# githubpradeep/llm_np_cp

Measured on AMD Instinct MI355X. Metric: decode tokens/sec, higher is better.
Workload: dtype bf16; 1 GPU; model=llama-3.2-1b, kv_dtype=bf16, global_batch=1, seq_len=867, parallelism=tp1

## Files before the change

### csrc/llm_ops.hip

```cpp

#include <hip/hip_runtime.h>
#include <cstdint>
#include <cstdio>
#include <cstdlib>
#include <type_traits>

#include "common.h"


#define GEMV_ROWS_PER_BLOCK 4
#define STAGE_RAW 0
#define STAGE_NORM 1
#define STAGE_GLU 2
#define STAGE_NORM2 3
#define STAGE_NORM_EMBED 4

DEVINL u16 glu_act(float xx, float u, int act) {
  float a;
  if (act == 0) {
    a = xx / (1.f + __expf(-xx));
  } else {
    float c = 0.7978845608028654f * (xx + 0.044715f * xx * xx * xx);
    a = 0.5f * xx * (1.f + tanhf(c));
  }
// ... 1605 lines not shown
        if (mnew != -INFINITY) mrun = mnew;
        kv = kvn; vv = vvn; kraw = krawn; vraw = vrawn;
        valid = validn; ksc = kscn; vsc = vscn;
      }
    }
  }

  for (int w = LP; w < 64; w <<= 1) {
    float mo = __shfl_xor(mrun, w);
    float lo = __shfl_xor(lrun, w);
    float mn = fmaxf(mrun, mo);
    float sa = (mrun == -INFINITY && mo == -INFINITY) ? 0.f : __expf(mrun - mn);
    float sb = (mrun == -INFINITY && mo == -INFINITY) ? 0.f : __expf(mo - mn);
#pragma unroll
    for (int j = 0; j < 8; j++) {
      float ao = __shfl_xor(acc[j], w);
      acc[j] = acc[j] * sa + ao * sb;
    }
    lrun = lrun * sa + lo * sb;
    mrun = mn;
  }

  float* accs = red;
  float* mls = red + 4 * hd;
  if (lane < LP) {
#pragma unroll
    for (int j = 0; j < 8; j++) accs[wave * hd + d0 + j] = acc[j];
  }
  if (lane == 0) {
    mls[wave * 2] = mrun;
    mls[wave * 2 + 1] = lrun;
  }
  __syncthreads();
  if (wave == 0) {
    float mt = fmaxf(fmaxf(mls[0], mls[2]), fmaxf(mls[4], mls[6]));
    float lt = 0.f, sc[4];
#pragma unroll
    for (int w = 0; w < 4; w++) {
      sc[w] = (mls[w * 2] == -INFINITY) ? 0.f : __expf(mls[w * 2] - mt);
      lt += mls[w * 2 + 1] * sc[w];
    }
    float inv = 1.f / lt;
    for (int d = lane; d < hd; d += 64) {
      float v = 0.f;
#pragma unroll
      for (int w = 0; w < 4; w++) v += accs[w * hd + d] * sc[w];
      out[((size_t)m * nh + h) * hd + d] = f2b(v * inv);
    }
  }
}


template <bool KV8>
__global__ void __launch_bounds__(256)
k_attn_dec_t(const u16* __restrict__ qkv, void* __restrict__ kc,
             void* __restrict__ vc, u16* __restrict__ out,
             const int* __restrict__ len_ptr, const float* __restrict__ cost,
             const float* __restrict__ sint, float* __restrict__ kS,
             float* __restrict__ vS, float* __restrict__ scratch,
             int* __restrict__ cnt, int nh, int kvh, int hd, int S,
             float scale, float softcap, int window) {
  extern __shared__ __attribute__((aligned(16))) char smem[];
  float* red = (float*)smem;
  int* lastflag = (int*)(red + 4 * hd + 8);

  const int h = blockIdx.x;
  const int chunk = blockIdx.y, SPLIT = gridDim.y;
  const int b = blockIdx.z;
  qkv += (size_t)b * (nh + 2 * kvh) * hd;
  out += (size_t)b * nh * hd;
  kc = (char*)kc + (size_t)b * kvh * S * hd * (KV8 ? 1 : 2);
  vc = (char*)vc + (size_t)b * kvh * S * hd * (KV8 ? 1 : 2);
  if (KV8) { kS += (size_t)b * kvh * S; vS += (size_t)b * kvh * S; }
  scratch += (size_t)b * nh * SPLIT * (hd + 2);
  cnt += b * nh;
  const int grp = nh / kvh;
  const int kvhead = h / grp;
  const int pos = len_ptr[b];
  int start = 0;
  if (window > 0 && pos + 1 - window > 0) start = pos + 1 - window;
  const int hist = pos - start;
  const int clen = (hist + SPLIT - 1) / SPLIT;
  const int c0 = start + chunk * clen;
  const int c1 = min(c0 + clen, pos);
  const bool last_chunk = (chunk == SPLIT - 1);

  const int LP = hd / 8;
  const int PP = 64 / LP;
  const int wave = threadIdx.x >> 6, lane = threadIdx.x & 63;
  const int p = lane / LP, d0 = (lane % LP) * 8;
  const int hd2 = hd / 2;
  const float* cp = cost + (size_t)pos * hd2;
  const float* sp = sint + (size_t)pos * hd2;

  const u16* qh = qkv + (size_t)h * hd;
  const u16* kh = qkv + (size_t)(nh + kvhead) * hd;
  const u16* vh = qkv + (size_t)(nh + kvh + kvhead) * hd;
  const u16* K0 = (const u16*)kc + (size_t)kvhead * S * hd;
  const u16* V0 = (const u16*)vc + (size_t)kvhead * S * hd;
  const uint8_t* K08 = (const uint8_t*)kc + (size_t)kvhead * S * hd;
  const uint8_t* V08 = (const uint8_t*)vc + (size_t)kvhead * S * hd;
  const float* kS0 = KV8 ? kS + (size_t)kvhead * S : nullptr;
  const float* vS0 = KV8 ? vS + (size_t)kvhead * S : nullptr;

  auto ldkv = [&](int tt, bool& vld, s8v& ko, s8v& vo,
                  unsigned long long& kro, unsigned long long& vro,
                  float& kso, float& vso) {
    vld = false;
    if (tt < c1) {
      int t_ = tt + p;
      vld = t_ < c1;
      int tl_ = vld ? t_ : c0;
      if (KV8) {
        kro = *(const unsigned long long*)(K08 + (size_t)tl_ * hd + d0);
        vro = *(const unsigned long long*)(V08 + (size_t)tl_ * hd + d0);
        kso = kS0[tl_]; vso = vS0[tl_];
      } else {
        ko = *(const s8v*)(K0 + (size_t)tl_ * hd + d0);
        vo = *(const s8v*)(V0 + (size_t)tl_ * hd + d0);
      }
// ... 190 lines not shown
    } else {
      for (int d = lane; d < hd; d += 64) {
        float v = 0.f;
#pragma unroll
        for (int w = 0; w < 4; w++) v += accs[w * hd + d] * sc[w];
        part[2 + d] = v;
      }
      if (lane == 0) { part[0] = mt; part[1] = lt; }
    }
  }
  if (SPLIT == 1) return;

  asm volatile("s_waitcnt vmcnt(0)" ::: "memory");
  __syncthreads();
  if (threadIdx.x == 0) {
    __builtin_amdgcn_fence(__ATOMIC_RELEASE, "agent");
    asm volatile("s_waitcnt vmcnt(0)" ::: "memory");
    int t = __hip_atomic_fetch_add(&cnt[h], 1, __ATOMIC_RELAXED,
                                   __HIP_MEMORY_SCOPE_AGENT);
    *lastflag = (t == SPLIT - 1);
  }
  __syncthreads();
  if (!*lastflag) return;

  if (threadIdx.x == 0)
    __builtin_amdgcn_fence(__ATOMIC_ACQUIRE, "agent");
  __syncthreads();
  if (wave == 0) {
    const float* base = scratch + (size_t)h * SPLIT * (hd + 2);
    float mt = -INFINITY;
    for (int c = 0; c < SPLIT; c++)
      mt = fmaxf(mt, base[(size_t)c * (hd + 2)]);
    float lt = 0.f;
    for (int c = 0; c < SPLIT; c++) {
      float mc = base[(size_t)c * (hd + 2)];
      if (mc != -INFINITY)
        lt += base[(size_t)c * (hd + 2) + 1] * __expf(mc - mt);
    }
    float inv = 1.f / lt;
    for (int d = lane; d < hd; d += 64) {
      float v = 0.f;
      for (int c = 0; c < SPLIT; c++) {
        float mc = base[(size_t)c * (hd + 2)];
        if (mc != -INFINITY)
          v += base[(size_t)c * (hd + 2) + 2 + d] * __expf(mc - mt);
      }
      out[(size_t)h * hd + d] = f2b(v * inv);
    }
  }
  __syncthreads();
  if (threadIdx.x == 0) cnt[h] = 0;
}

extern "C" hipError_t launch_attn_dec(const void* qkv, void* kc, void* vc,
                                      void* out, const void* len_ptr,
                                      const void* cost, const void* sint,
                                      void* kS, void* vS, int kv8,
                                      void* scratch, void* cnt, int split,
                                      int batch,
                                      int nh, int kvh, int hd, int S,
                                      float scale, float softcap, int window,
                                      hipStream_t stream) {
  size_t lds = (4 * hd + 8) * sizeof(float) + 16;
#define ATTN_DEC_CASE(KV8V)                                                  \
  hipLaunchKernelGGL((k_attn_dec_t<KV8V>), dim3(nh, split, batch),          \
                     dim3(256), lds,                                        \
                     stream, (const u16*)qkv, kc, vc, (u16*)out,            \
                     (const int*)len_ptr, (const float*)cost,               \
                     (const float*)sint, (float*)kS, (float*)vS,            \
                     (float*)scratch, (int*)cnt, nh, kvh, hd, S, scale,     \
                     softcap, window)
  if (kv8) ATTN_DEC_CASE(true);
  else ATTN_DEC_CASE(false);
#undef ATTN_DEC_CASE
  return hipGetLastError();
}


typedef short b4v __attribute__((ext_vector_type(4)));

template <int HD, bool KV8>
__global__ void __launch_bounds__(64)
k_attn_prefill_mfma(const u16* __restrict__ q, const void* __restrict__ kc,
                    const void* __restrict__ vc, u16* __restrict__ out,
                    const int* __restrict__ len_ptr,
                    const float* __restrict__ kS,
                    const float* __restrict__ vS, int M, int nh, int kvh,
                    int S, float scale, float softcap, int window) {
  constexpr int HD32 = HD / 32;
  constexpr int HD16 = HD / 16;
  const int h = blockIdx.x;
  const int qt = blockIdx.y;
  const int kvhead = h / (nh / kvh);
  const int pos0 = *len_ptr;
  const int lane = threadIdx.x & 63;
  const int qcol = lane & 15;
  const int krow4 = (lane >> 4) * 4;

  const int m0 = qt * 16;
  const int my_m = m0 + qcol;
  const int qpos = pos0 + my_m;

  s8v qf[HD32];
  {
    int mr = my_m < M ? my_m : M - 1;
    const u16* qp = q + ((size_t)mr * nh + h) * HD;
#pragma unroll
    for (int c = 0; c < HD32; c++)
      qf[c] = *(const s8v*)(qp + c * 32 + (lane >> 4) * 8);
  }

  const u16* K0 = (const u16*)kc + (size_t)kvhead * S * HD;
  const u16* V0 = (const u16*)vc + (size_t)kvhead * S * HD;
  const uint8_t* K08 = (const uint8_t*)kc + (size_t)kvhead * S * HD;
  const uint8_t* V08 = (const uint8_t*)vc + (size_t)kvhead * S * HD;
  const float* kS0 = KV8 ? kS + (size_t)kvhead * S : nullptr;
  const float* vS0 = KV8 ? vS + (size_t)kvhead * S : nullptr;

  float mrun = -INFINITY, lrun = 0.f;
  f4v acc_o[HD16];
#pragma unroll
  for (int d = 0; d < HD16; d++) acc_o[d] = {0.f, 0.f, 0.f, 0.f};

  __shared__ u16 vlds[16 * HD];
  const int T_end = min(pos0 + M, pos0 + m0 + 16);
  int t_start = 0;
  if (window > 0) {
    t_start = pos0 + m0 + 1 - window;
// ... 1571 lines not shown
#pragma unroll
  for (int i = 0; i < 4; i++) {
#pragma unroll
    for (int j = 0; j < 4; j++) {
#pragma unroll
      for (int r = 0; r < 4; r++) {
        int row = bm + wrow * 64 + i * 16 + cr + r;
        int col = bn + wcol * 64 + j * 16 + cc;
        if (row < M && col < N) {
          float v = acc[i][j][r];
          if (SK > 1) {
            atomicAdd(accbuf + (size_t)row * N + col, v);
          } else {
            if (res) v += b2f(res[(size_t)row * N + col]);
            Y[(size_t)row * N + col] = f2b(v);
          }
        }
      }
    }
  }
}

extern "C" hipError_t launch_gemm_fp4w(const void* X, const void* W4,
                                       const void* WE, void* Y,
                                       const void* res, void* accbuf, int M,
                                       int N, int K, hipStream_t stream) {
  if (K % 64 != 0) return hipErrorInvalidValue;
  int gm = (M + BM - 1) / BM, gn = (N + BN - 1) / BN;
  int sk = 1;
  if (accbuf && gm * gn < 160) {
    while (sk < 8 && gm * gn * sk * 2 <= 512 && (K / BK) % (sk * 2) == 0)
      sk *= 2;
  }
  if (sk > 1) {
    long total = (long)M * N;
    hipLaunchKernelGGL(k_zero_f32, dim3((uint32_t)((total + 1023) / 1024)),
                       dim3(256), 0, stream, (float*)accbuf, total);
  }
  dim3 grid(gm, gn, sk);
  hipLaunchKernelGGL(k_gemm_fp4w, grid, dim3(256), 0, stream, (const u16*)X,
                     (const uint8_t*)W4, (const uint8_t*)WE, (u16*)Y,
                     (const u16*)res, (float*)accbuf, M, N, K);
  if (sk > 1) {
    long total = (long)M * N;
    hipLaunchKernelGGL(k_gemm_fin, dim3((uint32_t)((total + 255) / 256)),
                       dim3(256), 0, stream, (const float*)accbuf,
                       (const u16*)res, (u16*)Y, total);
  }
  return hipGetLastError();
}


extern "C" __global__ void __launch_bounds__(256)
k_prefetch(const u16* __restrict__ p, long n, float* __restrict__ sink) {
  float acc = 0.f;
  for (long i = ((long)blockIdx.x * 256 + threadIdx.x) * 8; i < n;
       i += (long)gridDim.x * 256 * 8) {
    s8v v = *(const s8v*)(p + i);
    acc += b2f(((u16*)&v)[0]);
  }
  if (acc == 1e30f) sink[blockIdx.x] = acc;
}

extern "C" hipError_t launch_prefetch(const void* p, long n_elems,
                                      void* sink, hipStream_t stream) {
  hipLaunchKernelGGL(k_prefetch, dim3(128), dim3(256), 0, stream,
                     (const u16*)p, n_elems, (float*)sink);
  return hipGetLastError();
}


extern "C" __global__ void __launch_bounds__(256)
k_softcap(u16* __restrict__ y, long total, float cap) {
  long i = ((long)blockIdx.x * 256 + threadIdx.x) * 8;
  if (i >= total) return;
  s8v v = *(const s8v*)(y + i);
  u16 o[8];
#pragma unroll
  for (int j = 0; j < 8; j++)
    o[j] = f2b(cap * tanhf(b2f(((u16*)&v)[j]) / cap));
  *(s8v*)(y + i) = *(s8v*)o;
}

extern "C" hipError_t launch_softcap(void* y, long total, float cap,
                                     hipStream_t stream) {
  long blocks = (total / 8 + 255) / 256;
  hipLaunchKernelGGL(k_softcap, dim3((uint32_t)blocks), dim3(256), 0, stream,
                     (u16*)y, total, cap);
  return hipGetLastError();
}


extern "C" __global__ void __launch_bounds__(256)
k_bias_add(u16* __restrict__ y, const u16* __restrict__ bias, long total,
           int N) {
  long i = ((long)blockIdx.x * 256 + threadIdx.x) * 8;
  if (i >= total) return;
  s8v yv = *(const s8v*)(y + i);
  s8v bv = *(const s8v*)(bias + (i % N));
  u16 o[8];
#pragma unroll
  for (int j = 0; j < 8; j++)
    o[j] = f2b(b2f(((u16*)&yv)[j]) + b2f(((u16*)&bv)[j]));
  *(s8v*)(y + i) = *(s8v*)o;
}

extern "C" hipError_t launch_bias_add(void* y, const void* bias, int M,
                                      int N, hipStream_t stream) {
  if (N % 8 != 0) return hipErrorInvalidValue;
  long total = (long)M * N;
  hipLaunchKernelGGL(k_bias_add, dim3((uint32_t)((total / 8 + 255) / 256)),
                     dim3(256), 0, stream, (u16*)y, (const u16*)bias, total,
                     N);
  return hipGetLastError();
}


extern "C" __global__ void __launch_bounds__(256)
k_addinto(u16* __restrict__ y, const u16* __restrict__ a, long total) {
  long i = ((long)blockIdx.x * 256 + threadIdx.x) * 8;
  if (i >= total) return;
  s8v yv = *(const s8v*)(y + i);
  s8v av = *(const s8v*)(a + i);
  u16 o[8];
#pragma unroll
// ... 179 lines not shown
```

### llm_np_cp_amd/models/engine.py

```python

from __future__ import annotations

from typing import Dict, Optional

import numpy as np
import torch

from ..core.config import ModelConfig
from ..ops import hip_ops as ho
from ..parallel import tp as tpu
from ..utils.tracing import trace_range


class DeviceCacheHandle:

    def __init__(self, engine):
        self.engine = engine
        self.seq_len = 0


class GPUModel:
    device_strategies = frozenset(
        {"greedy", "min_p", "top_k", "top_p", "temperature"})
    device_processors = frozenset()
# ... 36 lines not shown
                {"logit_bias", "repetition_penalty", "frequency_penalty",
                 "presence_penalty"})
        self.p_stat = self.p_proc = self.p_bias = None
        self._proc_rows = {}
        if self.world == 1:
            self.device_logprobs = ho.LOGPROBS_MAX_TOP
        self.lp_cfg = self.lp_stage = self.lp_part = None
        self.lp_val = self.lp_idx = self.lp_raw = None
        self._lp_rows = {}
        self._lp_batch = False
        self.last_logprobs = None
        if self.world == 1:
            self.device_row_sampler = True
        self._samp_modes = {}
        self._req_serial = 0
        self._s_rows = frozenset({0})
        if device is None:
            device = f"cuda:{self.rank % max(torch.cuda.device_count(), 1)}"
        self.device = torch.device(device)
        torch.cuda.set_device(self.device)

        cfg = config
        tp = self.world
        assert cfg.num_attention_heads % tp == 0, "nh must divide tp"
        assert cfg.num_key_value_heads % tp == 0, \
            f"kv heads {cfg.num_key_value_heads} not divisible by tp {tp}"
        assert cfg.intermediate_size % tp == 0
        assert cfg.vocab_size % tp == 0
        if self.moe and tp > 1:
            raise ValueError("MoE tensor parallelism (expert parallel) "
                             "is not implemented yet — run TP=1")
        self.nh_l = cfg.num_attention_heads // tp
        self.kvh_l = cfg.num_key_value_heads // tp
        self.inter_l = cfg.intermediate_size // tp
        self.vocab_l = cfg.vocab_size // tp
        self.hd = cfg.head_dim
        self.H = cfg.hidden_size

        if self.world > 1:
            slot_bytes = max(self.H * 2, self.vocab_l * 4, 1 << 16)
            tpu.init_xgmi(self.device, slot_bytes)
        import torch.distributed as dist
        self._async_ar = bool(
            self.world > 1 and dist.is_initialized()
            and "nccl" in str(dist.get_backend()).lower())

        self._upload_weights(weights)
        if max_seq is None:
            max_seq = self._auto_max_seq()
        self.max_seq = max_seq
        self._alloc_state(prefill_chunk)
        self._graph = None
        self._graph_mode = None
        import os as _os
        self.prefetch_on = _os.environ.get("LLM_PREFETCH", "0") == "1"
        self._pf_stream = torch.cuda.Stream(device=self.device)
        self._pf_sink = torch.zeros(256, dtype=torch.float32,
                                    device=self.device)
        self._pf_events = []

    def _auto_max_seq(self) -> int:
        cfg = self.config
        free, _total = torch.cuda.mem_get_info(self.device)
        esz = 1 if self.kv8 else 2
        per_pos = (cfg.num_hidden_layers * self.kvh_l * self.hd * 2 * esz
                   * self.max_batch)
        if self.kv8:
            per_pos += (cfg.num_hidden_layers * self.kvh_l * 2 * 4
                        * self.max_batch)
        per_pos += self.hd * 4 + 8
        budget = int(free * 0.9) - (2 << 30)
        n = max(1024, budget // max(per_pos, 1))
        return int(min(cfg.max_position_embeddings, n))

    def _upload_weights(self, w: Dict[str, np.ndarray]):
        from ..io.loader import validate_weights

        validate_weights(self.config, w)
        cfg, dev = self.config, self.device
        tp, r = self.world, self.rank
        gemma = cfg.model_type == "gemma2"

        def bf16(a: np.ndarray) -> torch.Tensor:
            return torch.from_numpy(np.ascontiguousarray(a)).to(
                dev, torch.bfloat16, non_blocking=False)

        def gamma(a: np.ndarray) -> torch.Tensor:
            g = a.astype(np.float32) + (1.0 if gemma else 0.0)
            return torch.from_numpy(g).to(dev)

        def quant4(a: np.ndarray):
            t = bf16(a)
            N, K = t.shape
            q = torch.empty(N, K // 2, dtype=torch.uint8, device=dev)
            e = torch.empty(N, K // 32, dtype=torch.uint8, device=dev)
            ho.quant_fp4(t, q, e)
            torch.cuda.synchronize()
            return q, e

        def quant8(a: np.ndarray):
            t = bf16(a)
            N, K = t.shape
            q = torch.empty(N, K, dtype=torch.uint8, device=dev)
            s = torch.empty(N, dtype=torch.float32, device=dev)
            ho.quant_fp8(t, q, s)
            torch.cuda.synchronize()
            return q, s

        self.embed = bf16(w["model.embed_tokens.weight"])
        lm_w = w.get("lm_head.weight", w["model.embed_tokens.weight"])
        if self.fp8:
            lmw = lm_w if tp == 1 else tpu.shard_rows(lm_w, r, tp)
# ... 800 lines not shown
                if on_ids:
                    on_ids(take)
                if stop:
                    break
                if stop_fn is not None and stop_fn(out):
                    break
        if logprobs is not None:
            N = int(logprobs)
            self.last_logprobs = (
                np.concatenate([r[0] for r in recs]) if recs
                else np.zeros(0, np.float32),
                np.concatenate([r[1] for r in recs]) if recs
                else np.zeros((0, N), np.int32),
                np.concatenate([r[2] for r in recs]) if recs
                else np.zeros((0, N), np.float32))
        return out

    def forward(self, ids: np.ndarray, cache: DeviceCacheHandle,
                pos0: int) -> np.ndarray:
        ids = np.asarray(ids, dtype=np.int32).ravel()
        if pos0 != cache.seq_len:
            raise ValueError("GPU engine requires sequential positions")
        n = len(ids)
        if n == 0:
            raise ValueError("empty ids")
        if pos0 + n > self.max_seq:
            raise ValueError(f"sequence {pos0}+{n} exceeds max_seq "
                             f"{self.max_seq}")
        done = 0
        while done < n:
            M = min(n - done, self.PC)
            self.ids_buf[:M].copy_(
                torch.from_numpy(ids[done:done + M].astype(np.int32)))
            ho.i32_set(self.len_buf, pos0 + done)
            ho.embed(self.embed, self.ids_buf, self.b_h, M,
                     self.config.embed_scale)
            self._layers_forward(M)
            done += M
        ho.i32_set(self.len_buf, pos0 + n)
        self._host_len = pos0 + n
        self._lm_head_last(M)
        cache.seq_len = pos0 + n
        torch.cuda.synchronize()
        return self.b_logits.float().cpu().numpy()[None, :]

    def _dgemv(self, lw, name, x, y, **kw):
        if self.wq4:
            ho.gemv_fp4(lw[name + "_q4"], lw[name + "_e4"], x, y, **kw)
        elif self.fp8:
            ho.gemv_fp8(lw[name + "_q"], lw[name + "_s"], x, y, **kw)
        else:
            ho.gemv(lw[name], x, y, **kw)

    def _pf_tensors(self, lw):
        if self.wq4:
            return (lw["wqkv_q4"], lw["wo_q4"], lw["wgu_q4"],
                    lw["wdown_q4"])
        if self.fp8:
            return (lw["wqkv_q"], lw["wo_q"], lw["wgu_q"], lw["wdown_q"])
        return (lw["wqkv"], lw["wo"], lw["wgu"], lw["wdown"])

    def _decode_step(self, greedy: bool, min_p: float,
                     temperature: float = 1.0, top_k: int = 0,
                     top_p: float = 1.0, proc: bool = False,
                     logprobs: bool = False, rows=None):
        cfg = self.config
        eps = cfg.rms_norm_eps
        if self.fp8 or self.wq4:
            gukw = {}
            downkw = dict(stage=ho.STAGE_GLU, x2=self.b_gu[self.inter_l:],
                          act=self.act)
        else:
            gukw = dict(glu_pair=True, act=self.act)
            downkw = {}
        h = self.b_h[0]
        hnext = self.b_hb
        t1 = self.b_t1[0]
        t2 = self.b_t2
        s0 = torch.cuda.current_stream()
        pf = self.prefetch_on
        self._pf_events = []
        prev = None
        for i, lw in enumerate(self.layers):
            if pf and i + 1 < len(self.layers):
                ev = torch.cuda.Event()
                ev.record(s0)
                self._pf_events.append(ev)
                self._pf_stream.wait_event(ev)
                with torch.cuda.stream(self._pf_stream):
                    for t in self._pf_tensors(self.layers[i + 1]):
                        ho.prefetch(t, self._pf_sink)
            window = cfg.sliding_window if cfg.is_sliding(i) else 0
            if self.gemma and prev is not None:
                self._dgemv(lw, "wqkv", t2, self.b_qkv,
                            stage=ho.STAGE_NORM2, x2=h,
                            g=prev["g_postffn"], g2=lw["g_in"], res=hnext,
                            eps=eps)
                h, hnext = hnext, h
            elif i == 0 and "bqkv" not in lw:
                self._dgemv(lw, "wqkv", self.embed, self.b_qkv,
                            stage=ho.STAGE_NORM_EMBED, x2=self.next_token,
                            g=lw["g_in"], res=h, eps=eps,
                            escale=cfg.embed_scale)
            else:
                if i == 0:
                    ho.embed(self.embed, self.next_token, self.b_h, 1,
                             cfg.embed_scale)
                self._dgemv(lw, "wqkv", h, self.b_qkv, stage=ho.STAGE_NORM,
                            g=lw["g_in"], res=lw.get("bqkv"), eps=eps)
            prev = lw
            ho.attn_dec(self.b_qkv, self.k_cache[i], self.v_cache[i],
                        self.b_att[0], self.len_buf, self.cos_t, self.sin_t,
                        self.attn_scratch, self.attn_cnt,
                        self.nh_l, self.kvh_l, self.hd, self.scale,
                        softcap=self.attn_softcap, window=window or 0,
                        split=self.attn_split,
                        kS=self.k_scale[i], vS=self.v_scale[i])
            if self.gemma:
                self._dgemv(lw, "wo", self.b_att[0], t1)
                tpu.all_reduce(t1)
                self._dgemv(lw, "wgu", t1, self.b_gu, stage=ho.STAGE_NORM2,
                            x2=h, g=lw["g_post"], g2=lw["g_preffn"],
                            res=hnext, eps=eps, **gukw)
                h, hnext = hnext, h
                self._dgemv(lw, "wdown", self.b_gu[:self.inter_l], t2,
                            **downkw)
                tpu.all_reduce(t2)
            else:
                if self.tp_branch:
                    self._dgemv(lw, "wo", self.b_att[0], t1)
                    tpu.all_reduce(t1)
                    ho.addinto(h, t1)
                else:
                    self._dgemv(lw, "wo", self.b_att[0], h, res=h)
                if self.moe:
                    ho.moe_route(h, lw["g_post"], lw["wg"], 1, self.topk,
                                 self.moe_idx, self.moe_w, eps=eps)
                    xn0 = self.b_xn[0]
                    ho.rmsnorm(h, lw["g_post"], xn0, eps=eps)
                    I, H = self.inter_l, self.H
                    for j in range(self.topk):
                        ei = self.moe_idx[j:j + 1]
                        osc = self.moe_w[j:j + 1]
                        if self.fp8:
                            ho.gemv_fp8(lw["wgu_q"], lw["wgu_s"], xn0,
                                        self.b_gu, eidx=ei,
                                        wstride=2 * I * H, sstride=2 * I)
                            ho.gemv_fp8(lw["wdown_q"], lw["wdown_s"],
                                        self.b_gu[:I], h, res=h,
                                        stage=ho.STAGE_GLU,
                                        x2=self.b_gu[I:], act=self.act,
                                        eidx=ei, wstride=H * I,
                                        sstride=H, oscale=osc)
                        else:
                            ho.gemv(lw["wgu"], xn0, self.b_gu, eidx=ei,
                                    wstride=2 * I * H)
                            ho.gemv(lw["wdown"], self.b_gu[:I], h, res=h,
                                    stage=ho.STAGE_GLU, x2=self.b_gu[I:],
                                    act=self.act, eidx=ei,
                                    wstride=H * I, oscale=osc)
                    continue
                self._dgemv(lw, "wgu", h, self.b_gu, stage=ho.STAGE_NORM,
                            g=lw["g_post"], eps=eps, **gukw)
                if self.tp_branch:
                    self._dgemv(lw, "wdown", self.b_gu[:self.inter_l], t1,
                                **downkw)
                    tpu.all_reduce(t1)
                    ho.addinto(h, t1)
                else:
                    self._dgemv(lw, "wdown", self.b_gu[:self.inter_l], h,
                                res=h, **downkw)
        if pf:
            ev = torch.cuda.Event()
            ev.record(self._pf_stream)
            self._pf_events.append(ev)
            s0.wait_event(ev)
        if self.gemma:
            kw = dict(stage=ho.STAGE_NORM2, x2=h,
                      g=self.layers[-1]["g_postffn"], g2=self.g_final,
                      res=hnext, eps=eps, softcap=self.final_softcap)
            if self.wq4:
                ho.gemv_fp4(self.lm_head_q4, self.lm_head_e4, t2,
                            self.b_logits_l, **kw)
            elif self.fp8:
                ho.gemv_fp8(self.lm_head_q, self.lm_head_s, t2,
                            self.b_logits_l, **kw)
            else:
                ho.gemv(self.lm_head, t2, self.b_logits_l, **kw)
        else:
            kw = dict(stage=ho.STAGE_NORM, g=self.g_final, eps=eps,
                      softcap=self.final_softcap)
            if self.wq4:
                ho.gemv_fp4(self.lm_head_q4, self.lm_head_e4, h,
                            self.b_logits_l, **kw)
            elif self.fp8:
                ho.gemv_fp8(self.lm_head_q, self.lm_head_s, h,
                            self.b_logits_l, **kw)
            else:
                ho.gemv(self.lm_head, h, self.b_logits_l, **kw)
        if self.tp_branch:
            tpu.all_gather_into(self.b_logits, self.b_logits_l)
        if logprobs:
            self._lp_scan(self.b_logits, slice(0, 1), proc)
        if proc:
            ho.logit_adjust(self.b_logits, self.p_stat, self.p_proc,
                            self.p_bias, self.next_token, True)
        self._sample_step(greedy, min_p, temperature, top_k, top_p, rows)
        if logprobs:
            self._lp_commit(self.b_logits, slice(0, 1), proc,
                            self.next_token, self.nout)

    def _decode_batch_step(self, B: int, greedy: bool, min_p: float,
                           temperature: float = 1.0, top_k: int = 0,
                           top_p: float = 1.0, proc: bool = False,
                           logprobs: bool = False, rows=None):
        cfg = self.config
        import os as _os
        mx_max = int(_os.environ.get("LLM_BATCH_MX_MAX", "0"))
        if (self.fp8 and B <= mx_max and not cfg.attention_bias
                and not self.moe):
            return self._decode_batch_step_mx(B, greedy, min_p, temperature,
                                              top_k, top_p, proc, logprobs,
                                              rows)
        if self.fp8 and B <= 16 and not self.moe:
            return self._decode_batch_step_skinny(B, greedy, min_p,
                                                  temperature, top_k,
                                                  top_p, proc, logprobs,
                                                  rows)
        ho.embed(self.embed, self.bt_next, self.b_h, B, cfg.embed_scale)
# ... 604 lines not shown
```

### llm_np_cp_amd/ops/hip_ops.py

```python

from __future__ import annotations

import ctypes
import os

import numpy as np
import torch

_LIB = None
_LIB_PATH = os.path.join(os.path.dirname(os.path.dirname(
    os.path.abspath(__file__))), "_libllmops.so")

_SIGS = {
    "launch_gemv_bf16": [ctypes.c_void_p] * 7 + [ctypes.c_int] * 4 +
                        [ctypes.c_float, ctypes.c_int, ctypes.c_float,
                         ctypes.c_int, ctypes.c_int, ctypes.c_int,
                         ctypes.c_float, ctypes.c_void_p, ctypes.c_long,
                         ctypes.c_void_p, ctypes.c_void_p, ctypes.c_int],
    "launch_gemv_fp8": [ctypes.c_void_p] * 8 + [ctypes.c_int] * 4 +
                       [ctypes.c_float, ctypes.c_int, ctypes.c_float,
                        ctypes.c_int, ctypes.c_int, ctypes.c_int,
                        ctypes.c_float, ctypes.c_void_p, ctypes.c_long,
                        ctypes.c_long, ctypes.c_void_p, ctypes.c_void_p],
    "launch_rmsnorm": [ctypes.c_void_p] * 4 + [ctypes.c_int] * 2 +
                      [ctypes.c_float, ctypes.c_int, ctypes.c_void_p],
    "launch_rope_cache": [ctypes.c_void_p] * 7 + [ctypes.c_int] +
                         [ctypes.c_void_p] * 3 + [ctypes.c_int] * 5 +
                         [ctypes.c_void_p],
    "launch_attn": [ctypes.c_void_p] * 7 + [ctypes.c_int] * 6 +
                   [ctypes.c_float, ctypes.c_float, ctypes.c_int,
                    ctypes.c_void_p],
    "launch_attn_prefill_mfma": [ctypes.c_void_p] * 7 + [ctypes.c_int] * 6 +
                                [ctypes.c_float, ctypes.c_float,
                                 ctypes.c_int, ctypes.c_void_p],
    "launch_attn_dec": [ctypes.c_void_p] * 9 + [ctypes.c_int] +
                       [ctypes.c_void_p] * 2 + [ctypes.c_int] * 6 +
                       [ctypes.c_float, ctypes.c_float, ctypes.c_int,
                        ctypes.c_void_p],
    "launch_glu": [ctypes.c_void_p] * 3 + [ctypes.c_long, ctypes.c_int,
                                           ctypes.c_void_p],
    "launch_embed": [ctypes.c_void_p] * 3 + [ctypes.c_int] * 2 +
                    [ctypes.c_float, ctypes.c_void_p],
    "launch_sample": [ctypes.c_void_p, ctypes.c_int, ctypes.c_int,
                      ctypes.c_int, ctypes.c_long, ctypes.c_float,
                      ctypes.c_int, ctypes.c_uint64, ctypes.c_float] +
                     [ctypes.c_void_p] * 8 +
                     [ctypes.c_int, ctypes.c_void_p],
    "launch_sample_sel": [ctypes.c_void_p, ctypes.c_int, ctypes.c_int,
                          ctypes.c_int, ctypes.c_long, ctypes.c_float,
                          ctypes.c_int, ctypes.c_uint64, ctypes.c_float] +
                         [ctypes.c_void_p] * 8 +
                         [ctypes.c_int, ctypes.c_int, ctypes.c_float,
                          ctypes.c_void_p, ctypes.c_void_p],
    "launch_sample_rows": [ctypes.c_void_p, ctypes.c_int, ctypes.c_int,
                           ctypes.c_int, ctypes.c_long, ctypes.c_void_p,
                           ctypes.c_int, ctypes.c_int] +
                          [ctypes.c_void_p] * 7 +
                          [ctypes.c_int, ctypes.c_void_p, ctypes.c_void_p],
    "launch_logit_adjust": [ctypes.c_void_p, ctypes.c_int, ctypes.c_int,
                            ctypes.c_int] + [ctypes.c_void_p] * 4 +
                           [ctypes.c_int, ctypes.c_void_p],
    "launch_tokstat_mark": [ctypes.c_void_p, ctypes.c_void_p, ctypes.c_int,
                            ctypes.c_int, ctypes.c_void_p],
    "launch_logprob_scan": [ctypes.c_void_p, ctypes.c_int, ctypes.c_int,
                            ctypes.c_int, ctypes.c_void_p, ctypes.c_void_p,
                            ctypes.c_long] + [ctypes.c_void_p] * 3,
    "launch_logprob_commit": [ctypes.c_void_p, ctypes.c_int, ctypes.c_int,
                              ctypes.c_int] + [ctypes.c_void_p] * 8,
    "launch_gemm_bf16": [ctypes.c_void_p] * 5 + [ctypes.c_int] * 3 +
                        [ctypes.c_void_p],
    "launch_prefetch": [ctypes.c_void_p, ctypes.c_long, ctypes.c_void_p,
                        ctypes.c_void_p],
    "launch_softcap": [ctypes.c_void_p, ctypes.c_long, ctypes.c_float,
                       ctypes.c_void_p],
    "launch_addinto": [ctypes.c_void_p, ctypes.c_void_p, ctypes.c_long,
                       ctypes.c_void_p],
    "launch_bias_add": [ctypes.c_void_p, ctypes.c_void_p, ctypes.c_int,
                        ctypes.c_int, ctypes.c_void_p],
    "launch_i32_set": [ctypes.c_void_p, ctypes.c_int, ctypes.c_void_p],
    "launch_quant_fp8": [ctypes.c_void_p] * 3 + [ctypes.c_int] * 2 +
                        [ctypes.c_void_p],
    "launch_quant_fp4": [ctypes.c_void_p] * 3 + [ctypes.c_int] * 2 +
                        [ctypes.c_void_p],
    "launch_gemv_fp4": [ctypes.c_void_p] * 8 + [ctypes.c_int] * 4 +
                       [ctypes.c_float, ctypes.c_int, ctypes.c_float,
                        ctypes.c_int, ctypes.c_int, ctypes.c_int,
                        ctypes.c_float, ctypes.c_void_p],
    "launch_stage_quant_mx": [ctypes.c_void_p, ctypes.c_long,
                              ctypes.c_void_p, ctypes.c_long] +
                             [ctypes.c_void_p] * 4 +
                             [ctypes.c_void_p, ctypes.c_long] +
                             [ctypes.c_int] * 4 +
                             [ctypes.c_float, ctypes.c_float,
                              ctypes.c_void_p],
    "launch_gemm_fp8_skinny": [ctypes.c_void_p] * 5 + [ctypes.c_long] +
                              [ctypes.c_void_p, ctypes.c_long] +
                              [ctypes.c_void_p, ctypes.c_void_p,
                               ctypes.c_int,
                               ctypes.c_float] + [ctypes.c_int] * 3 +
                              [ctypes.c_void_p],
    "launch_gemv_fp8_mx": [ctypes.c_void_p] * 3 + [ctypes.c_long] +
                          [ctypes.c_void_p, ctypes.c_long] +
                          [ctypes.c_void_p] * 3 + [ctypes.c_long] +
                          [ctypes.c_void_p, ctypes.c_long] +
                          [ctypes.c_void_p, ctypes.c_long] +
                          [ctypes.c_int] * 5 +
                          [ctypes.c_float, ctypes.c_int, ctypes.c_float,
                           ctypes.c_float, ctypes.c_void_p],
    "launch_gemm_fp8": [ctypes.c_void_p] * 7 + [ctypes.c_int] * 3 +
                       [ctypes.c_void_p],
    "launch_gemm_fp4w": [ctypes.c_void_p] * 6 + [ctypes.c_int] * 3 +
                        [ctypes.c_void_p],
    "launch_moe_route": [ctypes.c_void_p] * 3 + [ctypes.c_int] * 4 +
                        [ctypes.c_float] + [ctypes.c_void_p] * 4,
    "launch_moe_scale_add": [ctypes.c_void_p] * 3 +
                            [ctypes.c_long, ctypes.c_int, ctypes.c_int,
                             ctypes.c_void_p],
    "launch_xgmi_coll": [ctypes.c_void_p, ctypes.c_void_p, ctypes.c_void_p,
                         ctypes.c_int, ctypes.c_int, ctypes.c_long,
                         ctypes.c_long, ctypes.c_int, ctypes.c_int,
                         ctypes.c_long, ctypes.c_void_p],
    "xc_alloc": [ctypes.c_long, ctypes.c_void_p],
    "xc_free": [ctypes.c_void_p],
    "xc_memset": [ctypes.c_void_p, ctypes.c_int, ctypes.c_long],
    "xc_h2d": [ctypes.c_void_p, ctypes.c_void_p, ctypes.c_long],
# ... 107 lines not shown
    S = k_cache.shape[1]
    _check(lib().launch_rope_cache(
        _ptr(q), _ptr(k_in), _ptr(v_in), _ptr(k_cache), _ptr(v_cache),
        _ptr(kS), _ptr(vS), 1 if kS is not None else 0,
        _ptr(cos_t), _ptr(sin_t), _ptr(pos_ptr), M, nh, kvh, hd, S,
        _stream()), "rope_cache")


def attn(q: torch.Tensor, k_cache: torch.Tensor, v_cache: torch.Tensor,
         out: torch.Tensor, len_ptr: torch.Tensor, M: int, nh: int,
         kvh: int, hd: int, scale: float, softcap: float = 0.0,
         window: int = 0, kS: torch.Tensor | None = None,
         vS: torch.Tensor | None = None):
    S = k_cache.shape[1]
    _check(lib().launch_attn(
        _ptr(q), _ptr(k_cache), _ptr(v_cache), _ptr(out), _ptr(len_ptr),
        _ptr(kS), _ptr(vS), 1 if kS is not None else 0,
        M, nh, kvh, hd, S, ctypes.c_float(scale), ctypes.c_float(softcap),
        window, _stream()), "attn")


def attn_prefill_mfma(q: torch.Tensor, k_cache: torch.Tensor,
                      v_cache: torch.Tensor, out: torch.Tensor,
                      len_ptr: torch.Tensor, M: int, nh: int, kvh: int,
                      hd: int, scale: float, softcap: float = 0.0,
                      window: int = 0, kS: torch.Tensor | None = None,
                      vS: torch.Tensor | None = None):
    S = k_cache.shape[1]
    _check(lib().launch_attn_prefill_mfma(
        _ptr(q), _ptr(k_cache), _ptr(v_cache), _ptr(out), _ptr(len_ptr),
        _ptr(kS), _ptr(vS), 1 if kS is not None else 0,
        M, nh, kvh, hd, S, ctypes.c_float(scale), ctypes.c_float(softcap),
        window, _stream()), "attn_prefill_mfma")


def attn_dec(qkv: torch.Tensor, k_cache: torch.Tensor,
             v_cache: torch.Tensor, out: torch.Tensor,
             len_ptr: torch.Tensor, cos_t: torch.Tensor,
             sin_t: torch.Tensor, scratch: torch.Tensor,
             cnt: torch.Tensor, nh: int, kvh: int, hd: int,
             scale: float, softcap: float = 0.0, window: int = 0,
             split: int = 1, kS: torch.Tensor | None = None,
             vS: torch.Tensor | None = None, batch: int = 1):
    S = k_cache.shape[-2]
    _check(lib().launch_attn_dec(
        _ptr(qkv), _ptr(k_cache), _ptr(v_cache), _ptr(out), _ptr(len_ptr),
        _ptr(cos_t), _ptr(sin_t), _ptr(kS), _ptr(vS),
        1 if kS is not None else 0,
        _ptr(scratch), _ptr(cnt), split, batch,
        nh, kvh, hd, S, ctypes.c_float(scale),
        ctypes.c_float(softcap), window, _stream()), "attn_dec")


def glu(gate: torch.Tensor, up: torch.Tensor, out: torch.Tensor, act: int):
    total = gate.numel()
    assert total % 8 == 0
    _check(lib().launch_glu(_ptr(gate), _ptr(up), _ptr(out), total, act,
                            _stream()), "glu")


def embed(table: torch.Tensor, ids: torch.Tensor, out: torch.Tensor,
          M: int, scale: float = 1.0):
    H = table.shape[1]
    _check(lib().launch_embed(_ptr(table), _ptr(ids), _ptr(out), M, H,
                              ctypes.c_float(scale), _stream()), "embed")


SAMPLE_SEL_WORDS = 260


def sample(logits: torch.Tensor, min_p: float, greedy: bool, seed: int,
           ctr: torch.Tensor, gmax: torch.Tensor, pick: torch.Tensor,
           next_token: torch.Tensor, out_ring: torch.Tensor,
           nout: torch.Tensor, len_ptr: torch.Tensor,
           bump_len: bool = True, temperature: float = 1.0,
           cnt: torch.Tensor | None = None, batch: int = 1, *,
           top_k: int = 0, top_p: float = 1.0,
           sel: torch.Tensor | None = None):
    if top_k < 0:
        raise ValueError(f"top_k must be >= 0, got {top_k}")
    if not 0.0 < top_p <= 1.0:
        raise ValueError(f"top_p must be in (0, 1], got {top_p}")
    filtered = top_k > 0 or top_p < 1.0
    if filtered and greedy:
        raise ValueError("top_k / top_p do not combine with greedy")
    if top_k > 0 and top_p < 1.0:
        raise ValueError("top_k and top_p are separate strategies; "
                         "pass one of them")
    if filtered and (sel is None or sel.dtype != torch.int64
                     or sel.numel() < batch * SAMPLE_SEL_WORDS):
        raise ValueError(f"top_k / top_p need an int64 `sel` scratch of "
                         f"{SAMPLE_SEL_WORDS} words per row")
    V = logits.shape[-1]
    lbf16 = 1 if logits.dtype == torch.bfloat16 else 0
    ring_stride = out_ring.shape[-1] if out_ring.dim() > 1 else 0
    if batch > 1:
        assert (gmax.numel() >= batch and pick.numel() >= batch
                and next_token.numel() >= batch and nout.numel() >= batch
                and cnt is not None and cnt.numel() >= batch)
    if cnt is None:
        global _SAMPLE_CNT
        try:
            _SAMPLE_CNT
        except NameError:
            _SAMPLE_CNT = {}
        key = logits.device
# ... 332 lines not shown
    _check(lib().launch_gemv_fp8_mx(
        _ptr(Wq), _ptr(scales), _ptr(x), ctypes.c_long(xstride),
        _ptr(x2), ctypes.c_long(x2stride), _ptr(g), _ptr(g2),
        _ptr(y), ctypes.c_long(ystride), _ptr(res), ctypes.c_long(rstride),
        _ptr(hout), ctypes.c_long(hstride), N, K, B, stage, act,
        ctypes.c_float(eps), out_f32, ctypes.c_float(softcap),
        ctypes.c_float(escale), _stream()), "gemv_fp8_mx")


def stage_quant_mx(x: torch.Tensor, xstride: int, xq: torch.Tensor,
                   sx: torch.Tensor, B: int, K: int, stage: int = 0,
                   x2: torch.Tensor | None = None, x2stride: int = 0,
                   g: torch.Tensor | None = None,
                   g2: torch.Tensor | None = None,
                   hout: torch.Tensor | None = None, hstride: int = 0,
                   act: int = 0, eps: float = 1e-5, escale: float = 1.0):
    _check(lib().launch_stage_quant_mx(
        _ptr(x), ctypes.c_long(xstride), _ptr(x2), ctypes.c_long(x2stride),
        _ptr(g), _ptr(g2), _ptr(xq), _ptr(sx), _ptr(hout),
        ctypes.c_long(hstride), K, B, stage, act, ctypes.c_float(eps),
        ctypes.c_float(escale), _stream()), "stage_quant_mx")


def gemm_fp8_skinny(xq: torch.Tensor, sx: torch.Tensor, Wq: torch.Tensor,
                    sw: torch.Tensor, y: torch.Tensor, B: int,
                    ystride: int, res: torch.Tensor | None = None,
                    rstride: int = 0, bias: torch.Tensor | None = None,
                    softcap: float = 0.0,
                    accbuf: torch.Tensor | None = None):
    N, K = Wq.shape
    out_f32 = 1 if y.dtype == torch.float32 else 0
    if accbuf is not None and accbuf.numel() < B * N:
        accbuf = None
    _check(lib().launch_gemm_fp8_skinny(
        _ptr(xq), _ptr(sx), _ptr(Wq), _ptr(sw), _ptr(y),
        ctypes.c_long(ystride), _ptr(res), ctypes.c_long(rstride),
        _ptr(bias), _ptr(accbuf), out_f32, ctypes.c_float(softcap),
        B, N, K, _stream()), "gemm_fp8_skinny")


def gemm_fp4w(X: torch.Tensor, Wq4: torch.Tensor, We4: torch.Tensor,
              Y: torch.Tensor, res: torch.Tensor | None = None,
              accbuf: torch.Tensor | None = None):
    M, K = X.shape
    N = Wq4.shape[0]
    assert Wq4.shape[1] * 2 == K and K % 64 == 0
    if accbuf is not None and accbuf.numel() < M * N:
        accbuf = None
    _check(lib().launch_gemm_fp4w(
        _ptr(X), _ptr(Wq4), _ptr(We4), _ptr(Y), _ptr(res), _ptr(accbuf),
        M, N, K, _stream()), "gemm_fp4w")


def prefetch(t: torch.Tensor, sink: torch.Tensor):
    n = t.numel() * t.element_size() // 2
    _check(lib().launch_prefetch(_ptr(t), n, _ptr(sink), _stream()),
           "prefetch")


def softcap(y: torch.Tensor, cap: float):
    total = y.numel()
    assert total % 8 == 0
    _check(lib().launch_softcap(_ptr(y), total, ctypes.c_float(cap),
                                _stream()), "softcap")


def bias_add(y: torch.Tensor, bias: torch.Tensor, M: int):
    N = bias.numel()
    _check(lib().launch_bias_add(_ptr(y), _ptr(bias), M, N, _stream()),
           "bias_add")


def addinto(y: torch.Tensor, a: torch.Tensor):
    total = y.numel()
    assert total % 8 == 0
    _check(lib().launch_addinto(_ptr(y), _ptr(a), total, _stream()), "addinto")


def i32_set(buf: torch.Tensor, v: int):
    _check(lib().launch_i32_set(_ptr(buf), v, _stream()), "i32_set")



XC_MODE_AR_BF16, XC_MODE_AR_F32, XC_MODE_GATHER = 0, 1, 2
XC_OFF_EPOCH, XC_OFF_TICKET, XC_OFF_ERR = 64, 72, 76
XC_OFF_DATA = 4096
XC_IPC_HANDLE_BYTES = 64


def xc_alloc(nbytes: int) -> int:
    p = ctypes.c_void_p(0)
    _check(lib().xc_alloc(ctypes.c_long(nbytes), ctypes.byref(p)), "xc_alloc")
    return p.value


def xc_free(ptr: int):
    _check(lib().xc_free(ctypes.c_void_p(ptr)), "xc_free")


def xc_memset(ptr: int, val: int, nbytes: int):
    _check(lib().xc_memset(ctypes.c_void_p(ptr), val,
                           ctypes.c_long(nbytes)), "xc_memset")


def xc_h2d(dst: int, data: bytes):
    buf = (ctypes.c_char * len(data)).from_buffer_copy(data)
    _check(lib().xc_h2d(ctypes.c_void_p(dst), buf,
                        ctypes.c_long(len(data))), "xc_h2d")


def xc_d2h(src: int, nbytes: int) -> bytes:
    buf = (ctypes.c_char * nbytes)()
# ... 51 lines not shown
```

Baseline: 1355 tokens/s.

## Prefetch next o-proj weights into cache from extra attention-decode blocks

Adds extra thread blocks to the decode attention launch. These blocks, rather than computing attention, read the upcoming wo (and optionally wgu) weight regions so they land in the last-level cache while attention runs. The read pattern for wo mirrors the consumer GEMV's block stride so lines match the XCD-local consumers. This replaces the old, env-gated side-stream prefetch kernel, which is removed. The new path is on by default ('auto' budget up to 10MB). The cost is extra memory traffic and blocks competing with the latency-bound attention kernel.

```diff
diff --git a/csrc/llm_ops.hip b/csrc/llm_ops.hip
--- a/csrc/llm_ops.hip
+++ b/csrc/llm_ops.hip
@@ -1681,20 +1681,20 @@
 
 
 template <bool KV8>
-__global__ void __launch_bounds__(256)
-k_attn_dec_t(const u16* __restrict__ qkv, void* __restrict__ kc,
-             void* __restrict__ vc, u16* __restrict__ out,
-             const int* __restrict__ len_ptr, const float* __restrict__ cost,
-             const float* __restrict__ sint, float* __restrict__ kS,
-             float* __restrict__ vS, float* __restrict__ scratch,
-             int* __restrict__ cnt, int nh, int kvh, int hd, int S,
-             float scale, float softcap, int window) {
-  extern __shared__ __attribute__((aligned(16))) char smem[];
+DEVINL void attn_dec_body(char* smem, const int chunk, const int SPLIT,
+                          const u16* __restrict__ qkv, void* __restrict__ kc,
+                          void* __restrict__ vc, u16* __restrict__ out,
+                          const int* __restrict__ len_ptr,
+                          const float* __restrict__ cost,
+                          const float* __restrict__ sint,
+                          float* __restrict__ kS, float* __restrict__ vS,
+                          float* __restrict__ scratch, int* __restrict__ cnt,
+                          int nh, int kvh, int hd, int S, float scale,
+                          float softcap, int window) {
   float* red = (float*)smem;
   int* lastflag = (int*)(red + 4 * hd + 8);
 
   const int h = blockIdx.x;
-  const int chunk = blockIdx.y, SPLIT = gridDim.y;
   const int b = blockIdx.z;
   qkv += (size_t)b * (nh + 2 * kvh) * hd;
   out += (size_t)b * nh * hd;
@@ -1991,6 +1991,157 @@
   if (threadIdx.x == 0) cnt[h] = 0;
 }
 
+
+struct AttnPf {
+  const void* ptr[4];
+  long bytes[4];
+  long stride0;
+  float* sink;
+  int never;
+};
+
+constexpr int PF_LD = 8;
+constexpr int PF_TRIP = 256 * PF_LD;
+
+template <typename F>
+DEVINL uint32_t attn_pf_trip(const u4v* __restrict__ base, long nseg, F seg) {
+  u4v v[PF_LD];
+#pragma unroll
+  for (int j = 0; j < PF_LD; j++) {
+    long s = seg(j * 256 + (int)threadIdx.x);
+    s = s < nseg ? s : nseg - 1;
+    v[j] = base[s];
+  }
+  uint32_t a = 0;
+#pragma unroll
+  for (int j = 0; j < PF_LD; j++) {
+    asm volatile("" ::"v"(v[j]));
+    a ^= v[j][0];
+  }
+  return a;
+}
+
+DEVINL void attn_dec_prefetch(const AttnPf& pf, const int split) {
+  const uint32_t nx = gridDim.x;
+  const uint32_t pfy = gridDim.y - split;
+  const uint32_t npb = nx * pfy * gridDim.z;
+  const uint32_t pb =
+      (blockIdx.z * pfy + (blockIdx.y - split)) * nx + blockIdx.x;
+  uint32_t acc = 0;
+  uint32_t g0 = 0;
+#pragma unroll
+  for (int r = 0; r < 4; r++) {
+    const u4v* base = (const u4v*)pf.ptr[r];
+    const long nseg = pf.bytes[r] >> 4;
+    if (base == nullptr || nseg <= 0) continue;
+    const long spu = pf.stride0 >> 4;
+    if (r == 0 && spu > 0 && (nx & 7) == 0 && nseg < (1l << 31)) {
+      const uint32_t c = blockIdx.x & 7;
+      const uint32_t nunit = (uint32_t)((nseg + spu - 1) / spu);
+      if (nunit <= c) continue;
+      const uint32_t uspu = (uint32_t)spu;
+      const long vseg = (long)((nunit - c + 7) / 8) * spu;
+      const uint32_t rc = (pb / nx) * (nx / 8) + blockIdx.x / 8;
+      for (long t = rc; t * PF_TRIP < vseg; t += npb / 8) {
+        acc ^= attn_pf_trip(base, nseg, [&](int i) {
+          long v = t * PF_TRIP + i;
+          v = v < vseg ? v : vseg - 1;
+          const uint32_t k = (uint32_t)v / uspu;
+          return (long)(c + 8 * k) * spu + ((uint32_t)v - k * uspu);
+        });
+      }
+      continue;
+    }
+    const long ntrip = (nseg + PF_TRIP - 1) / PF_TRIP;
+    for (long t = (pb + npb - g0) % npb; t < ntrip; t += npb)
+      acc ^= attn_pf_trip(base, nseg,
+                          [&](int i) { return t * PF_TRIP + i; });
+    g0 = (uint32_t)((g0 + ntrip) % npb);
+  }
+  asm volatile("" ::"v"(acc));
+  asm volatile("s_waitcnt vmcnt(0)" ::: "memory");
+  if ((int)threadIdx.x == pf.never) pf.sink[pb & 255] = (float)acc;
+}
+
+struct AttnPfLaunch {
+  int split;
+  AttnPf pf;
+};
+
+template <bool KV8, bool PF, typename... PFA>
+__global__ void __launch_bounds__(256)
+k_attn_dec_t(const u16* __restrict__ qkv, void* __restrict__ kc,
+             void* __restrict__ vc, u16* __restrict__ out,
+             const int* __restrict__ len_ptr, const float* __restrict__ cost,
+             const float* __restrict__ sint, float* __restrict__ kS,
+             float* __restrict__ vS, float* __restrict__ scratch,
+             int* __restrict__ cnt, int nh, int kvh, int hd, int S,
+             float scale, float softcap, int window, PFA... pfa) {
+  static_assert(sizeof...(PFA) == (PF ? 1 : 0), "PF takes one AttnPfLaunch");
+  extern __shared__ __attribute__((aligned(16))) char smem[];
+  int SPLIT = gridDim.y;
+  if constexpr (PF) {
+    const AttnPfLaunch& a = (pfa, ...);
+    if ((int)blockIdx.y >= a.split) {
+      attn_dec_prefetch(a.pf, a.split);
+      return;
+    }
+    SPLIT = a.split;
+  }
+  attn_dec_body<KV8>(smem, blockIdx.y, SPLIT, qkv, kc, vc, out, len_ptr, cost,
+                     sint, kS, vS, scratch, cnt, nh, kvh, hd, S, scale,
+                     softcap, window);
+}
+
+static hipError_t attn_dec_launch(const void* qkv, void* kc, void* vc,
+                                  void* out, const void* len_ptr,
+                                  const void* cost, const void* sint,
+                                  void* kS, void* vS, int kv8, void* scratch,
+                                  void* cnt, int split, int batch, int nh,
+                                  int kvh, int hd, int S, float scale,
+                                  float softcap, int window, int pf_blocks,
+                                  const AttnPf& pf, hipStream_t stream) {
+  size_t lds = (4 * hd + 8) * sizeof(float) + 16;
+  const int pfy = pf_blocks > 0 ? (pf_blocks + nh - 1) / nh : 0;
+#define ATTN_DEC_ARGS                                                        \
+  (const u16*)qkv, kc, vc, (u16*)out, (const int*)len_ptr,                   \
+      (const float*)cost, (const float*)sint, (float*)kS, (float*)vS,        \
+      (float*)scratch, (int*)cnt, nh, kvh, hd, S, scale, softcap, window
+#define ATTN_DEC_CASE(KV8V)                                                  \
+  hipLaunchKernelGGL((k_attn_dec_t<KV8V, false>), dim3(nh, split, batch),    \
+                     dim3(256), lds, stream, ATTN_DEC_ARGS)
+#define ATTN_DEC_PF_CASE(KV8V)                                               \
+  hipLaunchKernelGGL((k_attn_dec_t<KV8V, true, AttnPfLaunch>),               \
+                     dim3(nh, split + pfy, batch), dim3(256), lds, stream,   \
+                     ATTN_DEC_ARGS, AttnPfLaunch{split, pf})
+  if (pfy > 0) {
+    if (kv8) ATTN_DEC_PF_CASE(true);
+    else ATTN_DEC_PF_CASE(false);
+  } else {
+    if (kv8) ATTN_DEC_CASE(true);
+    else ATTN_DEC_CASE(false);
+  }
+#undef ATTN_DEC_PF_CASE
+#undef ATTN_DEC_ARGS
+#undef ATTN_DEC_CASE
+  return hipGetLastError();
+}
+
+extern "C" hipError_t launch_attn_dec_pf(
+    const void* qkv, void* kc, void* vc, void* out, const void* len_ptr,
+    const void* cost, const void* sint, void* kS, void* vS, int kv8,
+    void* scratch, void* cnt, int split, int batch, int nh, int kvh, int hd,
+    int S, float scale, float softcap, int window, int pf_blocks,
+    const void* p0, long n0, const void* p1, long n1, const void* p2,
+    long n2, const void* p3, long n3, long stride0, void* sink,
+    hipStream_t stream) {
+  AttnPf pf{{p0, p1, p2, p3}, {n0, n1, n2, n3}, stride0, (float*)sink, -1};
+  if (pf_blocks > 0 && sink == nullptr) return hipErrorInvalidValue;
+  return attn_dec_launch(qkv, kc, vc, out, len_ptr, cost, sint, kS, vS, kv8,
+                         scratch, cnt, split, batch, nh, kvh, hd, S, scale,
+                         softcap, window, pf_blocks, pf, stream);
+}
+
 extern "C" hipError_t launch_attn_dec(const void* qkv, void* kc, void* vc,
                                       void* out, const void* len_ptr,
                                       const void* cost, const void* sint,
@@ -2000,19 +2151,9 @@
                                       int nh, int kvh, int hd, int S,
                                       float scale, float softcap, int window,
                                       hipStream_t stream) {
-  size_t lds = (4 * hd + 8) * sizeof(float) + 16;
-#define ATTN_DEC_CASE(KV8V)                                                  \
-  hipLaunchKernelGGL((k_attn_dec_t<KV8V>), dim3(nh, split, batch),          \
-                     dim3(256), lds,                                        \
-                     stream, (const u16*)qkv, kc, vc, (u16*)out,            \
-                     (const int*)len_ptr, (const float*)cost,               \
-                     (const float*)sint, (float*)kS, (float*)vS,            \
-                     (float*)scratch, (int*)cnt, nh, kvh, hd, S, scale,     \
-                     softcap, window)
-  if (kv8) ATTN_DEC_CASE(true);
-  else ATTN_DEC_CASE(false);
-#undef ATTN_DEC_CASE
-  return hipGetLastError();
+  return attn_dec_launch(qkv, kc, vc, out, len_ptr, cost, sint, kS, vS, kv8,
+                         scratch, cnt, split, batch, nh, kvh, hd, S, scale,
+                         softcap, window, 0, AttnPf{}, stream);
 }
 
 
@@ -3690,25 +3831,6 @@
 
 
 extern "C" __global__ void __launch_bounds__(256)
-k_prefetch(const u16* __restrict__ p, long n, float* __restrict__ sink) {
-  float acc = 0.f;
-  for (long i = ((long)blockIdx.x * 256 + threadIdx.x) * 8; i < n;
-       i += (long)gridDim.x * 256 * 8) {
-    s8v v = *(const s8v*)(p + i);
-    acc += b2f(((u16*)&v)[0]);
-  }
-  if (acc == 1e30f) sink[blockIdx.x] = acc;
-}
-
-extern "C" hipError_t launch_prefetch(const void* p, long n_elems,
-                                      void* sink, hipStream_t stream) {
-  hipLaunchKernelGGL(k_prefetch, dim3(128), dim3(256), 0, stream,
-                     (const u16*)p, n_elems, (float*)sink);
-  return hipGetLastError();
-}
-
-
-extern "C" __global__ void __launch_bounds__(256)
 k_softcap(u16* __restrict__ y, long total, float cap) {
   long i = ((long)blockIdx.x * 256 + threadIdx.x) * 8;
   if (i >= total) return;
diff --git a/llm_np_cp_amd/models/attn_prefetch.py b/llm_np_cp_amd/models/attn_prefetch.py
--- /dev/null
+++ b/llm_np_cp_amd/models/attn_prefetch.py
@@ -0,0 +1,45 @@
+
+from __future__ import annotations
+
+from typing import List, Tuple
+
+Region = Tuple[str, int, int]
+
+
+def _down16(n: int) -> int:
+    return max(0, int(n)) & ~15
+
+
+def plan_attn_prefetch(wo_bytes: int, wgu_bytes: int, I: int, K: int,
+                       budget: int, *, moe: bool = False) -> List[Region]:
+    if moe or budget <= 0:
+        return []
+    out: List[Region] = []
+    n_wo = _down16(min(wo_bytes, budget))
+    if n_wo:
+        out.append(("wo", 0, n_wo))
+    left = budget - wo_bytes
+    if left <= 0 or I <= 0 or wgu_bytes <= 0:
+        return out
+    row = wgu_bytes // (2 * I)
+    if row <= 0 or row % 16 or row * 2 * I != wgu_bytes:
+        return out
+    r = min(I, (left // 2) // row)
+    if r > 0:
+        out.append(("wgu", 0, r * row))
+        out.append(("wgu", I * row, r * row))
+    return out
+
+
+def consumer_stride(wo_bytes: int, n_rows: int, rows_per_block: int) -> int:
+    if n_rows <= 0 or wo_bytes % n_rows:
+        return 0
+    s = wo_bytes // n_rows * rows_per_block
+    return s if s % 16 == 0 else 0
+
+
+AUTO_MAX_BYTES = 10 << 20
+
+
+def default_budget(wo_bytes: int, wgu_bytes: int) -> int:
+    return wo_bytes if 0 < wo_bytes <= AUTO_MAX_BYTES else 0
diff --git a/llm_np_cp_amd/models/engine.py b/llm_np_cp_amd/models/engine.py
--- a/llm_np_cp_amd/models/engine.py
+++ b/llm_np_cp_amd/models/engine.py
@@ -112,12 +112,35 @@
         self._alloc_state(prefill_chunk)
         self._graph = None
         self._graph_mode = None
+        self._plan_attn_pf()
+
+    def _plan_attn_pf(self):
         import os as _os
-        self.prefetch_on = _os.environ.get("LLM_PREFETCH", "0") == "1"
-        self._pf_stream = torch.cuda.Stream(device=self.device)
-        self._pf_sink = torch.zeros(256, dtype=torch.float32,
-                                    device=self.device)
-        self._pf_events = []
+        from .attn_prefetch import (consumer_stride, default_budget,
+                                    plan_attn_prefetch)
+        self._attn_pf = None
+        _b = _os.environ.get("LLM_ATTN_PF", "auto").strip().lower()
+        if _b in ("", "0") or self.moe:
+            return
+        sfx = "_q4" if self.wq4 else "_q" if self.fp8 else ""
+        plans = []
+        for lw in self.layers:
+            wo, wgu = lw["wo" + sfx], lw["wgu" + sfx]
+            nb = {"wo": wo.numel() * wo.element_size(),
+                  "wgu": wgu.numel() * wgu.element_size()}
+            budget = (default_budget(nb["wo"], nb["wgu"]) if _b == "auto"
+                      else int(_b))
+            base = {"wo": wo.data_ptr(), "wgu": wgu.data_ptr()}
+            plans.append([(base[n] + off, size) for n, off, size in
+                          plan_attn_prefetch(nb["wo"], nb["wgu"],
+                                             self.inter_l, self.H, budget)])
+            self.attn_pf_stride = consumer_stride(nb["wo"], self.H, 4)
+        _n = _os.environ.get("LLM_ATTN_PF_BLOCKS")
+        self.attn_pf_blocks = int(_n) if _n else 4 * self.nh_l
+        if self.attn_pf_blocks > 0 and any(plans):
+            self._attn_pf = plans
+            self._pf_sink = torch.zeros(256, dtype=torch.float32,
+                                        device=self.device)
 
     def _auto_max_seq(self) -> int:
         cfg = self.config
@@ -1024,14 +1047,6 @@
         else:
             ho.gemv(lw[name], x, y, **kw)
 
-    def _pf_tensors(self, lw):
-        if self.wq4:
-            return (lw["wqkv_q4"], lw["wo_q4"], lw["wgu_q4"],
-                    lw["wdown_q4"])
-        if self.fp8:
-            return (lw["wqkv_q"], lw["wo_q"], lw["wgu_q"], lw["wdown_q"])
-        return (lw["wqkv"], lw["wo"], lw["wgu"], lw["wdown"])
-
     def _decode_step(self, greedy: bool, min_p: float,
                      temperature: float = 1.0, top_k: int = 0,
                      top_p: float = 1.0, proc: bool = False,
@@ -1049,19 +1064,8 @@
         hnext = self.b_hb
         t1 = self.b_t1[0]
         t2 = self.b_t2
-        s0 = torch.cuda.current_stream()
-        pf = self.prefetch_on
-        self._pf_events = []
         prev = None
         for i, lw in enumerate(self.layers):
-            if pf and i + 1 < len(self.layers):
-                ev = torch.cuda.Event()
-                ev.record(s0)
-                self._pf_events.append(ev)
-                self._pf_stream.wait_event(ev)
-                with torch.cuda.stream(self._pf_stream):
-                    for t in self._pf_tensors(self.layers[i + 1]):
-                        ho.prefetch(t, self._pf_sink)
             window = cfg.sliding_window if cfg.is_sliding(i) else 0
             if self.gemma and prev is not None:
                 self._dgemv(lw, "wqkv", t2, self.b_qkv,
@@ -1081,13 +1085,21 @@
                 self._dgemv(lw, "wqkv", h, self.b_qkv, stage=ho.STAGE_NORM,
                             g=lw["g_in"], res=lw.get("bqkv"), eps=eps)
             prev = lw
-            ho.attn_dec(self.b_qkv, self.k_cache[i], self.v_cache[i],
-                        self.b_att[0], self.len_buf, self.cos_t, self.sin_t,
-                        self.attn_scratch, self.attn_cnt,
-                        self.nh_l, self.kvh_l, self.hd, self.scale,
-                        softcap=self.attn_softcap, window=window or 0,
-                        split=self.attn_split,
-                        kS=self.k_scale[i], vS=self.v_scale[i])
+            pfkw = {}
+            attn_dec = ho.attn_dec
+            if self._attn_pf is not None and self._attn_pf[i]:
+                attn_dec = ho.attn_dec_pf
+                pfkw = dict(regions=self._attn_pf[i],
+                            pf_blocks=self.attn_pf_blocks,
+                            stride0=self.attn_pf_stride,
+                            sink=self._pf_sink)
+            attn_dec(self.b_qkv, self.k_cache[i], self.v_cache[i],
+                     self.b_att[0], self.len_buf, self.cos_t, self.sin_t,
+                     self.attn_scratch, self.attn_cnt,
+                     self.nh_l, self.kvh_l, self.hd, self.scale,
+                     softcap=self.attn_softcap, window=window or 0,
+                     split=self.attn_split,
+                     kS=self.k_scale[i], vS=self.v_scale[i], **pfkw)
             if self.gemma:
                 self._dgemv(lw, "wo", self.b_att[0], t1)
                 tpu.all_reduce(t1)
@@ -1142,11 +1154,6 @@
                 else:
                     self._dgemv(lw, "wdown", self.b_gu[:self.inter_l], h,
                                 res=h, **downkw)
-        if pf:
-            ev = torch.cuda.Event()
-            ev.record(self._pf_stream)
-            self._pf_events.append(ev)
-            s0.wait_event(ev)
         if self.gemma:
             kw = dict(stage=ho.STAGE_NORM2, x2=h,
                       g=self.layers[-1]["g_postffn"], g2=self.g_final,
diff --git a/llm_np_cp_amd/ops/hip_ops.py b/llm_np_cp_amd/ops/hip_ops.py
--- a/llm_np_cp_amd/ops/hip_ops.py
+++ b/llm_np_cp_amd/ops/hip_ops.py
@@ -37,6 +37,12 @@
                        [ctypes.c_void_p] * 2 + [ctypes.c_int] * 6 +
                        [ctypes.c_float, ctypes.c_float, ctypes.c_int,
                         ctypes.c_void_p],
+    "launch_attn_dec_pf": [ctypes.c_void_p] * 9 + [ctypes.c_int] +
+                          [ctypes.c_void_p] * 2 + [ctypes.c_int] * 6 +
+                          [ctypes.c_float, ctypes.c_float, ctypes.c_int,
+                           ctypes.c_int] +
+                          [ctypes.c_void_p, ctypes.c_long] * 4 +
+                          [ctypes.c_long, ctypes.c_void_p, ctypes.c_void_p],
     "launch_glu": [ctypes.c_void_p] * 3 + [ctypes.c_long, ctypes.c_int,
                                            ctypes.c_void_p],
     "launch_embed": [ctypes.c_void_p] * 3 + [ctypes.c_int] * 2 +
@@ -69,8 +75,6 @@
                               ctypes.c_int] + [ctypes.c_void_p] * 8,
     "launch_gemm_bf16": [ctypes.c_void_p] * 5 + [ctypes.c_int] * 3 +
                         [ctypes.c_void_p],
-    "launch_prefetch": [ctypes.c_void_p, ctypes.c_long, ctypes.c_void_p,
-                        ctypes.c_void_p],
     "launch_softcap": [ctypes.c_void_p, ctypes.c_long, ctypes.c_float,
                        ctypes.c_void_p],
     "launch_addinto": [ctypes.c_void_p, ctypes.c_void_p, ctypes.c_long,
@@ -284,6 +288,35 @@
         ctypes.c_float(softcap), window, _stream()), "attn_dec")
 
 
+def attn_dec_pf(qkv: torch.Tensor, k_cache: torch.Tensor,
+                v_cache: torch.Tensor, out: torch.Tensor,
+                len_ptr: torch.Tensor, cos_t: torch.Tensor,
+                sin_t: torch.Tensor, scratch: torch.Tensor,
+                cnt: torch.Tensor, nh: int, kvh: int, hd: int,
+                scale: float, softcap: float = 0.0, window: int = 0,
+                split: int = 1, kS: torch.Tensor | None = None,
+                vS: torch.Tensor | None = None, batch: int = 1, *,
+                regions=(), pf_blocks: int = 0, stride0: int = 0,
+                sink: torch.Tensor | None = None):
+    S = k_cache.shape[-2]
+    regions = list(regions)
+    assert len(regions) <= 4
+    if pf_blocks > 0:
+        assert sink is not None and sink.numel() >= 256
+    flat = []
+    for addr, nbytes in regions + [(0, 0)] * (4 - len(regions)):
+        assert addr % 16 == 0 and nbytes >= 0
+        flat += [addr, nbytes]
+    _check(lib().launch_attn_dec_pf(
+        _ptr(qkv), _ptr(k_cache), _ptr(v_cache), _ptr(out), _ptr(len_ptr),
+        _ptr(cos_t), _ptr(sin_t), _ptr(kS), _ptr(vS),
+        1 if kS is not None else 0,
+        _ptr(scratch), _ptr(cnt), split, batch,
+        nh, kvh, hd, S, ctypes.c_float(scale),
+        ctypes.c_float(softcap), window, pf_blocks, *flat, stride0,
+        _ptr(sink), _stream()), "attn_dec_pf")
+
+
 def glu(gate: torch.Tensor, up: torch.Tensor, out: torch.Tensor, act: int):
     total = gate.numel()
     assert total % 8 == 0
@@ -722,12 +755,6 @@
         M, N, K, _stream()), "gemm_fp4w")
 
 
-def prefetch(t: torch.Tensor, sink: torch.Tensor):
-    n = t.numel() * t.element_size() // 2
-    _check(lib().launch_prefetch(_ptr(t), n, _ptr(sink), _stream()),
-           "prefetch")
-
-
 def softcap(y: torch.Tensor, cap: float):
     total = y.numel()
     assert total % 8 == 0
```

Result: faster. 1374 tokens/s (median of 6 runs) (+1.4%).
